# yeyupiaoling/PPASR

Hardware: AMD Instinct MI355X
Metric: audio-seconds/s (RTF^-1) Conformer-streaming fbank, batch32 per GPU, ctc_greedy (higher is better)
Workload: dtype f32; 1 GPU; configs[1]: Conformer streaming (configs/conformer.yml), fbank-80, 32 x 10 s utterances per GPU, V=4233, ctc_greedy, features resident in HBM -> token ids + scores on device; global_batch=32, frames=1000, decoder=ctc_greedy, parallelism=utterance-dp1, pipelined=False, gemm=f32

## Files before the change

### ppasr_amd/csrc/conformer_kernels.hip

```cpp
#include <cstdlib>

#include "conformer_kernels.h"
#include "launch.h"
#include "phases.h"
#include "h3.h"

#include <math.h>

namespace ppasr {
#ifdef PPASR_PHASE_TS
}
extern "C" __attribute__((visibility("default"))) int ppasr_debug_read_phase_ts(long long* out) {
  return (int)hipMemcpyFromSymbol(out, HIP_SYMBOL(ppasr::g_phase_ts), sizeof(long long) * 128);
}
extern "C" __attribute__((visibility("default"))) int ppasr_debug_read_wave_ts(long long* out) {
  return (int)hipMemcpyFromSymbol(out, HIP_SYMBOL(ppasr::g_wave_ts), sizeof(long long) * 512);
}
extern "C" __attribute__((visibility("default"))) int ppasr_debug_read_wg_ts(long long* out) {
  return (int)hipMemcpyFromSymbol(out, HIP_SYMBOL(ppasr::g_wg_ts), sizeof(long long) * 2 * 1024);
}
namespace ppasr {
#endif


// ... 26 lines not shown
  }
};
struct QkvStoreSide {
  const f32x16& acc;
  float* out;
  const f32x4 (&bias)[4];
  __device__ __forceinline__ void operator()(int g) const {
    if ((g & 7) == 4 && out) {
      const int q = g >> 3;
      *reinterpret_cast<f32x4*>(out + 8 * q) = f32x4{acc[4 * q] + bias[q][0], acc[4 * q + 1] + bias[q][1],
                                                     acc[4 * q + 2] + bias[q][2], acc[4 * q + 3] + bias[q][3]};
    }
  }
};

template <bool H3 = false>
__device__ __forceinline__ void ffn_qkv_body(float* bufX, float* bufA, float* bufH, float* __restrict__ x1,
                                             float* __restrict__ qkv, const LayerW& w, int r0, int valid, int n_chunks,
                                             BRing<1>& ring, VtOut vt = VtOut{}) {
  const int lane = lane_id(), wave = wave_id();
  rb_layernorm(bufX, bufA, kLda, kRows, w.ln_mac_g, w.ln_mac_b, 1e-5f);
  __syncthreads();
  PPASR_TS(8);
  f32x16 acc2[1][1];
  acc_zero(acc2);
  const f32x4* wq = w.wqkv + (size_t)wave * kTs256;
  if constexpr (H3) ffn_phase_h3(bufA, w.ffm_w1, w.ffm_b1, w.ffm_w2, n_chunks, wq, ring, acc2);
  else ffn_phase<true>(bufA, bufH, w.ffm_w1, w.ffm_b1, w.ffm_w2, n_chunks, wq, ring, acc2);
  PPASR_TS(9);
  residual_epilogue_t(bufX, acc2, w.ffm_b2, 0.5f);
  __syncthreads();
  PPASR_TS(10);
  rb_store_rows(x1 + (size_t)r0 * kD, bufX, kLda, kRows, valid);
  rb_layernorm(bufX, bufA, kLda, kRows, w.ln_mha_g, w.ln_mha_b, 1e-5f);
  __syncthreads();
  if constexpr (H3) h3_planes_from_tile(bufA, reinterpret_cast<_Float16*>(bufA));
  PPASR_TS(11);
  f32x16 tile[3][1][1]; bool qk_bad = false;
  const int cq = wave * 32 + 4 * (lane >> 5);
  float* qrow = (lane & 31) < valid ? qkv + (size_t)(r0 + (lane & 31)) * 768 + cq : nullptr;
  f32x4 qb[2][4], kp[4];
#pragma unroll
  for (int c = 0; c < 3; ++c)
#pragma unroll
    for (int q = 0; q < 4; ++q) (c < 2 ? qb[c][q] : kp[q]) = qkv_bias_quad<H3>(w.bqkv, vt, c, r0 + (lane & 31), cq + 8 * q);
#pragma unroll
  for (int c = 0; c < 3; ++c) {
    acc_zero(tile[c]);
    const f32x4* seg = w.wqkv + (size_t)(c * 8 + wave) * kTs256;
    const f32x4* nseg = c < 2 ? seg + 8 * kTs256 : nullptr;
    if constexpr (H3) {
      const _Float16* pa = reinterpret_cast<const _Float16*>(bufA);
      if (c < 2)
        rb_gemm_h3(pa, seg, nseg, ring, tile[c][0][0]);
      else
        rb_gemm_h3_rows<1, 16, QkStoreTailH3>(pa, kLdh, kPlaneH, seg, nseg, ring, tile[c],
                                              QkStoreTailH3{tile[0][0][0], tile[1][0][0], qrow, qb, vt.k_h3 != 0, qk_bad, cq});
    } else if (c == 0) {
      rb_gemm<1, 1, kG256, kPF, NoSide, true>(bufA, kLda, seg, 0, nseg, 0, ring, tile[c]);
    } else if (c == 1) {
      rb_gemm<1, 1, kG256, kPF, QkvStoreSide, true>(bufA, kLda, seg, 0, nseg, 0, ring, tile[c],
                                                    QkvStoreSide{tile[0][0][0], qrow, qb[0]});
    } else {
      rb_gemm<1, 1, kG256, kPF, QkvStoreSide, false>(bufA, kLda, seg, 0, nseg, 0, ring, tile[c],
                                                     QkvStoreSide{tile[1][0][0], qrow ? qrow + 256 : nullptr, qb[1]});
    }
    if (c == 0) qkv_kpos_add<H3>(qb[1], kp, vt);
    PPASR_TS(12 + c);
  }
  if constexpr (H3) h3_note(qk_bad);
  if (vt.vt) {
    const float bv = w.bqkv[2 * 256 + wave * 32 + (lane & 31)];
    float* dst = vt.vt + ((size_t)wave * (vt.stride >> 3) + (r0 >> 3)) * 256 + 4 * lane;
    if constexpr (H3) tile[2][0][0] *= kH3Inv;
#pragma unroll
    for (int i = 0; i < 4; ++i) {
      const f32x16& t = tile[2][0][0];
      *reinterpret_cast<f32x4*>(dst + i * 256) = f32x4{t[4 * i] + bv, t[4 * i + 1] + bv, t[4 * i + 2] + bv, t[4 * i + 3] + bv};
    }
  } else {
    const int col = 2 * 256 + wave * 32 + (lane & 31);
    const float bv = w.bqkv[col];
    if constexpr (H3) tile[2][0][0] *= kH3Inv;
#pragma unroll
    for (int r = 0; r < 16; ++r) {
      int row = acc_row(r, lane);
      if (row < valid) qkv[(size_t)(r0 + row) * 768 + col] = tile[2][0][0][r] + bv;
    }
  }
}

__global__ __launch_bounds__(kThreads) void k_ffn_qkv(const float* __restrict__ x_in, float* __restrict__ x1,
                                                      float* __restrict__ qkv, LayerW w, int M, int n_chunks, PadSkip ps,
                                                      VtOut vt) {
  extern __shared__ __attribute__((aligned(16))) float smem[];
  const int blk = pad_block_of(ps, kRows, M);
  if (blk < 0) return;
  float* bufX = smem;
  float* bufA = bufX + kRows * kLda;
  float* bufH = bufA + kRows * kLda;
  const int wave = wave_id();
  const int r0 = blk * kRows;
  const int valid = min(kRows, M - r0);
  BRing<1> ring;
  ring_prime(ring, w.ffm_w1 + (size_t)wave * kTs256, 0);
  rb_load_rows(bufX, kLda, x_in + (size_t)r0 * kD, kRows, valid);
  ffn_qkv_body(bufX, bufA, bufH, x1, qkv, w, r0, valid, n_chunks, ring, vt);
}
__global__ __launch_bounds__(256) void k_repack_h3(const float* __restrict__ src, _Float16* __restrict__ dst, int n_tiles, int G,
                                                   unsigned int* __restrict__ ovf) {
  const int KS = G >> 1;
  const long long t = (long long)blockIdx.x * 256 + threadIdx.x;
  if (t >= (long long)n_tiles * KS * 64) return;
  const int l = (int)(t & 63), ks = (int)((t >> 6) % KS), nt = (int)((t >> 6) / KS);
  const float* g = src + ((size_t)nt * G + 2 * ks + (l >> 5)) * 256;
  f16x8 hi, lo;
#pragma unroll
  for (int e = 0; e < 8; ++e) {
    const float v = g[((l & 31) + 32 * (e >> 2)) * 4 + (e & 3)] * kH3Sw;
    if (!(fabsf(v) <= kH3Max)) atomicAdd(ovf, 1u);
    hi[e] = (_Float16)v;
    lo[e] = (_Float16)(v - (float)hi[e]);
// ... 29 lines not shown
__global__ __launch_bounds__(kThreads) void k_ffn_qkv_h3(const float* __restrict__ x_in, float* __restrict__ x1,
                                                         float* __restrict__ qkv, LayerW w, int M, int n_chunks, PadSkip ps,
                                                         VtOut vt) {
  extern __shared__ __attribute__((aligned(16))) float smem[];
  const int blk = pad_block_of(ps, kRows, M);
  if (blk < 0) return;
  float* bufX = smem;
  float* bufA = bufX + kRows * kLda;
  float* bufH = bufA + kRows * kLda;
  const int wave = wave_id();
  const int r0 = blk * kRows;
  const int valid = min(kRows, M - r0);
  BRing<1> ring;
  ring_prime(ring, w.ffm_w1 + (size_t)wave * kTs256, 0);
  rb_load_rows(bufX, kLda, x_in + (size_t)r0 * kD, kRows, valid);
  ffn_qkv_body<true>(bufX, bufA, bufH, x1, qkv, w, r0, valid, n_chunks, ring, vt);
}
static void check_form(const char* stage, int rows, bool only32) {
  if (rows == 32 || ((rows == 16 || rows == kW16) && !only32)) return;
  fprintf(stderr, "ppasr_hip: %s refused: row-block form %d%s\n", stage, rows,
          only32 ? " with h3, g_hist, xhat_out, split_xhat or hm (8-wave 32-row form only)" : " (32, 16 or kW16)");
  abort();
}
constexpr size_t kLdsFfnQkv = 4 * kRows * kLda * sizeof(float);
void launch_ffn_qkv(const float* x_in, float* x1, float* qkv, const LayerW& w, int M, int n_chunks, hipStream_t st,
                    const PadSkip& ps, VtOut vt, bool h3, int rows) {
  check_form("launch_ffn_qkv", rows, h3);
  if (rows == 16) return LayerStagesT<16>::ffn_qkv(x_in, x1, qkv, w, M, n_chunks, st, ps, VtOut{});
  if (rows == kW16) return LayerStagesT<kW16>::ffn_qkv(x_in, x1, qkv, w, M, n_chunks, st, ps, vt);
  if (h3) {
    PPASR_LAUNCH(k_ffn_qkv_h3, dim3((M + kRows - 1) / kRows), dim3(kThreads), kLdsFfnQkv + kH3ExtraLds, st, x_in, x1, qkv, w,
                 M, n_chunks, ps, vt);
    return;
  }
  PPASR_LAUNCH(k_ffn_qkv, dim3((M + kRows - 1) / kRows), dim3(kThreads), kLdsFfnQkv, st, x_in, x1, qkv, w, M,
                     n_chunks, ps, vt);
}

void launch_attention(const AttnArgs& a, int B, int H, hipStream_t st) {
// ... 135 lines not shown
  if (split_xhat) {
    if (h3)
      PPASR_LAUNCH(k_pw1_glu_cols<true>, dim3(grid.x, 2), dim3(kThreads), kLdsPw1Cols + 512, st, xh, g, w, M, ps);
    else
      PPASR_LAUNCH(k_pw1_glu_cols<false>, dim3(grid.x, 2), dim3(kThreads), kLdsPw1Cols, st, xh, g, w, M, ps);
  }
}

constexpr int kPLd = 68;
constexpr int kPTile = 32 * kPLd;
constexpr int kFusedAttnFloats = kWaves * kPTile + kWaves * 64 + kRows * kLda;
static_assert(2 * kRows * kLda <= kWaves * kPTile + kWaves * 64, "bufX/bufA alias the attention scratch");
static_assert(kRows * kLda + 128 + 4 * kPTile <= kWaves * kPTile, "the d rows (fp16 x3: the Q'_v planes, 512 B longer) and the four merge tiles fit in front of Stat");
static_assert(kH3TileBytes <= kRows * kLda * 4 + 512, "fp16 x3: the Q'_u planes at bufC run 512 B past it (the launch asks for them)");
static_assert(kRows * kLda * 4 + kH3TileBytes <= kWaves * kPTile * 4, "fp16 x3: operand planes at bufA stay in front of Stat");
static_assert(kFusedAttnFloats * 4 <= 160 * 1024, "LDS budget");
template <bool H3>
__device__ __forceinline__ void attn_out_glu_body(const AttnArgs& a, int B, const float* __restrict__ x1, float* __restrict__ x2,
                                                  float* __restrict__ g, const LayerW& w) {
  extern __shared__ __attribute__((aligned(16))) float smem[];
  float* Ps = smem;
  float* Stat = Ps + kWaves * kPTile;
  float* bufC = Stat + kWaves * 64;
  float* bufX = smem;
  float* bufA = bufX + kRows * kLda;
  const int lane = lane_id(), wave = wave_id();
  const int h = wave >> 1, khalf = wave & 1;
  const int nq = (a.T1 + 31) / 32;
  const int slot = blockIdx.x >> 3;
  const int b = (slot / nq) * 8 + (blockIdx.x & 7);
  const int q0 = (slot % nq) * 32;
  if (b >= B) return;
  const int T = a.T1;
  const int valid = min(32, T - q0);
  const float* __restrict__ qb = a.q + (size_t)b * T * a.q_stride;
  const float* __restrict__ kbp = a.k + (size_t)b * a.T2 * a.k_stride;
  const float* __restrict__ vbp = a.v + (size_t)b * a.T2 * a.v_stride;
  const float* __restrict__ ptab = a.ptab + (size_t)a.pos0 * kD;
  const int pstride = a.pos_stride;
  const int64_t len_b = a.lens ? a.lens[b] : (int64_t)a.mask_mul * a.T2;
// ... 65 lines not shown
      if constexpr (H3) {
        f16x4 hi, lo;
        h3_split4((v + pu) * kH3Sa, hi, lo, bad);
        _Float16* pu_pl = reinterpret_cast<_Float16*>(bufC) + row * kLdh + 4 * lane;
        *reinterpret_cast<f16x4*>(pu_pl) = hi;
        *reinterpret_cast<f16x4*>(pu_pl + kPlaneH) = lo;
        h3_split4((v + pv) * kH3Sa, hi, lo, bad);
        _Float16* pv_pl = reinterpret_cast<_Float16*>(QV) + row * kLdh + 4 * lane;
        *reinterpret_cast<f16x4*>(pv_pl) = hi;
        *reinterpret_cast<f16x4*>(pv_pl + kPlaneH) = lo;
      } else {
        *reinterpret_cast<f32x4*>(bufC + row * kLda + 4 * lane) = v + pu;
      }
    }
    if constexpr (H3) h3_note(bad);
    __syncthreads();
  }
  const float* qfrag_u = bufC + l31 * kLda + h * 64 + 4 * hh;
  auto qfrag = [&](int gk) -> f32x4 { return *reinterpret_cast<const f32x4*>(qfrag_u + 8 * gk); };
  PPASR_TS(33);
  if (khalf * 128 < U) prime_k(khalf * 128);
  f32x16 acc_o[2];
#pragma unroll
  for (int t = 0; t < 2; ++t)
#pragma unroll
    for (int r = 0; r < 16; ++r) acc_o[t][r] = 0.f;
  float m_run = -INFINITY, l_run = 0.f;
  bool first = true;

  const int nkb = (U + 255) / 256;
  for (int kb = 0; kb < nkb; ++kb) {
// ... 189 lines not shown
    if constexpr (!H3) {
#pragma unroll
      for (int q = 0; q < 4; ++q) res[q] = *reinterpret_cast<const f32x4*>(x1 + grow + cq + 8 * q);
    }
    f32x16 acc[1][1];
    acc_zero(acc);
    if constexpr (H3) {
      h3_planes_from_tile(bufC, reinterpret_cast<_Float16*>(bufA));
      rb_gemm_h3(reinterpret_cast<const _Float16*>(bufA), seg_o, seg_val, ring, acc[0][0]);
      acc[0][0] *= kH3Inv;
    } else {
      rb_gemm<1, 1, kG256, kPF, NoSide, true>(bufC, kLda, seg_o, 0, seg_val, 0, ring, acc);
    }
#pragma unroll
    for (int q = 0; q < 4; ++q) {
      const f32x4 bo = *reinterpret_cast<const f32x4*>(w.bo + cq + 8 * q);
      f32x4 v;
#pragma unroll
      for (int e = 0; e < 4; ++e) v[e] = res[q][e] + (acc[0][0][4 * q + e] + bo[e]);
      if constexpr (H3) x2v[q] = v;
      else if (row_ok) *reinterpret_cast<f32x4*>(x2 + grow + cq + 8 * q) = v;
      if (!row_ok) v = f32x4{0.f, 0.f, 0.f, 0.f};
      *reinterpret_cast<f32x4*>(bufX + l31 * kLda + cq + 8 * q) = v;
    }
  }
  __syncthreads();
  PPASR_TS(37);
  struct PadHere {
    int64_t len_b;
    int q0, mul;
    __device__ __forceinline__ bool operator()(int row) const { return (int64_t)mul * (q0 + row) >= len_b; }
  };
  rb_layernorm<false>(bufX, bufA, kLda, kRows, w.ln_conv_g, w.ln_conv_b, 1e-5f,
                      PadHere{a.lens ? len_b : (int64_t)1 << 62, q0, a.mask_mul});
  __syncthreads();
  PPASR_TS(38);
  {
    f32x16 av[1][1], ag[1][1];
    acc_zero(av);
    acc_zero(ag);
    if constexpr (H3) {
      h3_planes_from_tile(bufA, reinterpret_cast<_Float16*>(bufA));
      rb_gemm_h3(reinterpret_cast<const _Float16*>(bufA), seg_val, seg_gate, ring, av[0][0]);
      rb_gemm_h3(reinterpret_cast<const _Float16*>(bufA), seg_gate, nullptr, ring, ag[0][0]);
      av[0][0] *= kH3Inv;
      ag[0][0] *= kH3Inv;
    } else {
      rb_gemm<1, 1, kG256, kPF, NoSide, true>(bufA, kLda, seg_val, 0, seg_gate, 0, ring, av);
      rb_gemm<1, 1, kG256, kPF, NoSide, true>(bufA, kLda, seg_gate, 0, nullptr, 0, ring, ag);
    }
#pragma unroll
    for (int q = 0; q < 4; ++q) {
      const f32x4 bval = *reinterpret_cast<const f32x4*>(w.pw1_b + cq + 8 * q);
      const f32x4 bgate = *reinterpret_cast<const f32x4*>(w.pw1_b + kD + cq + 8 * q);
      const f32x2 s0 = sigmoid2(f32x2{ag[0][0][4 * q] + bgate[0], ag[0][0][4 * q + 1] + bgate[1]});
      const f32x2 s1 = sigmoid2(f32x2{ag[0][0][4 * q + 2] + bgate[2], ag[0][0][4 * q + 3] + bgate[3]});
      const f32x4 o = {(av[0][0][4 * q] + bval[0]) * s0[0], (av[0][0][4 * q + 1] + bval[1]) * s0[1],
                       (av[0][0][4 * q + 2] + bval[2]) * s1[0], (av[0][0][4 * q + 3] + bval[3]) * s1[1]};
      if (row_ok) *reinterpret_cast<f32x4*>(g + grow + cq + 8 * q) = o;
    }
    if constexpr (H3) {
      if (row_ok) {
#pragma unroll
        for (int q = 0; q < 4; ++q) *reinterpret_cast<f32x4*>(x2 + grow + cq + 8 * q) = x2v[q];
      }
    }
  }
  PPASR_TS(39);
  PPASR_WG_TS(512 + 1);
}
__global__ __launch_bounds__(kThreads) void k_attn_out_glu(AttnArgs a, int B, const float* __restrict__ x1,
                                                           float* __restrict__ x2, float* __restrict__ g, LayerW w) {
  attn_out_glu_body<false>(a, B, x1, x2, g, w);
}
__global__ __launch_bounds__(kThreads) void k_attn_out_glu_h3(AttnArgs a, int B, const float* __restrict__ x1,
                                                              float* __restrict__ x2, float* __restrict__ g, LayerW w) {
  attn_out_glu_body<true>(a, B, x1, x2, g, w);
}
constexpr size_t kLdsAttnOutGlu = (size_t)kFusedAttnFloats * sizeof(float);
void launch_attn_out_glu(const AttnArgs& a, int B, const float* x1, float* x2, float* g, const LayerW& w, hipStream_t st, bool h3) {
  const int nq = (a.T1 + 31) / 32;
  if (h3)
    PPASR_LAUNCH(k_attn_out_glu_h3, dim3(nq * ((B + 7) / 8) * 8), dim3(kThreads), kLdsAttnOutGlu + 512, st, a, B, x1, x2, g, w);
  else
    PPASR_LAUNCH(k_attn_out_glu, dim3(nq * ((B + 7) / 8) * 8), dim3(kThreads), kLdsAttnOutGlu, st, a, B, x1, x2, g, w);
}

template <int KS, bool STREAM, bool NEXT, bool H3>
__device__ __forceinline__ void conv_ffn_body(const float* __restrict__ g, const float* __restrict__ g_hist,
                                              const float* __restrict__ x2, float* __restrict__ x_out, const LayerW& w,
                                              const int64_t* __restrict__ lens, int M, int Tp, int n_chunks, int mask_mul,
                                              const LayerW& wn, float* __restrict__ x1_next, float* __restrict__ qkv_next,
                                              int left_ctx, const PadSkip& ps, VtOut vt_next) {
  extern __shared__ __attribute__((aligned(16))) float smem[];
  const int blk = pad_block_of(ps, kRows, M);
  if (blk < 0) return;
  float* bufX = smem;
  float* bufA = bufX + kRows * kLda;
  float* bufH = bufA + kRows * kLda;
  const int lane = lane_id(), wave = wave_id();
  const int r0 = blk * kRows;
  const int valid = min(kRows, M - r0);
  const int col = wave * 32 + (lane & 31);
  BRing<1> ring;
  const f32x4* seg_pw2 = w.pw2 + (size_t)wave * kTs256;
  PPASR_TS(0);
  if (NEXT) PPASR_WG_TS(0);
  ring_prime(ring, seg_pw2, 0);
  const int pb0 = r0 / Tp, pt0 = r0 - pb0 * Tp, pnb = max(M / Tp, 1);
  int64_t plen0 = 0, plen1 = 0;
  if (lens && Tp >= kRows) {
    plen0 = lens[min(pb0, pnb - 1)];
    plen1 = lens[min(pb0 + 1, pnb - 1)];
  }
  if (!STREAM && KS <= 15 && Tp >= kRows / kWaves) {
    if constexpr (!STREAM && KS <= 15)
      dwconv_ln_phase<KS>(g, bufA, w.dw_w, w.dw_b, w.glu_pad, w.ln_cm_g, w.ln_cm_b, w.cm_eps, r0, M, Tp, left_ctx);
    PPASR_TS(1);
// ... 10 lines not shown
    const float* rp = x2 + (size_t)(r0 + min(l31, valid - 1)) * kD + cq;
#pragma unroll
    for (int q = 0; q < 4; ++q) res[q] = *reinterpret_cast<const f32x4*>(rp + 8 * q);
  }
  bool pad = false;
  if (lens) {
    if (Tp >= kRows) {
      const int tt = pt0 + l31;
      const bool over = tt >= Tp;
      const int64_t t = over ? tt - Tp : tt, len = over ? plen1 : plen0;
      pad = r0 + l31 < M && (int64_t)mask_mul * t >= len;
    } else {
      pad = is_pad(l31);
    }
  }
  __syncthreads();
  PPASR_TS(2);
  {
    f32x16 acc[1][1];
    acc_zero(acc);
    if constexpr (H3) {
      h3_planes_from_tile(bufA, reinterpret_cast<_Float16*>(bufA));
      rb_gemm_h3(reinterpret_cast<const _Float16*>(bufA), seg_pw2, w.ff_w1 + (size_t)wave * kTs256, ring, acc[0][0]);
      acc[0][0] *= kH3Inv;
    } else {
      rb_gemm<1, 1, kG256, kPF, NoSide, true>(bufA, kLda, seg_pw2, 0, w.ff_w1 + (size_t)wave * kTs256, 0, ring, acc);
    }
#pragma unroll
    for (int q = 0; q < 4; ++q) {
      const f32x4 bv = *reinterpret_cast<const f32x4*>(w.pw2_b + cq + 8 * q);
      f32x4 o;
#pragma unroll
      for (int e = 0; e < 4; ++e) o[e] = (l31 < valid) ? res[q][e] + (pad ? 0.f : acc[0][0][4 * q + e] + bv[e]) : 0.f;
      *reinterpret_cast<f32x4*>(bufX + l31 * kLda + cq + 8 * q) = o;
    }
  }
  __syncthreads();
  PPASR_TS(3);
  rb_layernorm(bufX, bufA, kLda, kRows, w.ln_ff_g, w.ln_ff_b, 1e-5f);
  __syncthreads();
  PPASR_TS(4);
  f32x16 acc2[1][1];
  acc_zero(acc2);
  if constexpr (H3)
    ffn_phase_h3(bufA, w.ff_w1, w.ff_b1, w.ff_w2, n_chunks, NEXT ? wn.ffm_w1 + (size_t)wave * kTs256 : nullptr, ring, acc2);
  else
    ffn_phase<true>(bufA, bufH, w.ff_w1, w.ff_b1, w.ff_w2, n_chunks, NEXT ? wn.ffm_w1 + (size_t)wave * kTs256 : nullptr,
                    ring, acc2);
  PPASR_TS(5);
  residual_epilogue_t(bufX, acc2, w.ff_b2, 0.5f);
  __syncthreads();
  PPASR_TS(6);
  rb_layernorm(bufX, bufX, kLda, kRows, w.ln_fin_g, w.ln_fin_b, 1e-5f);
  if (x_out) rb_store_rows(x_out + (size_t)r0 * kD, bufX, kLda, kRows, valid);
  PPASR_TS(7);
  if (NEXT) ffn_qkv_body<H3>(bufX, bufA, bufH, x1_next, qkv_next, wn, r0, valid, n_chunks, ring, vt_next);
  PPASR_TS(15);
  if (NEXT) PPASR_WG_TS(1);
}
template <int KS, bool STREAM, bool NEXT>
__global__ __launch_bounds__(kThreads) void k_conv_ffn(const float* __restrict__ g, const float* __restrict__ g_hist,
                                                       const float* __restrict__ x2, float* __restrict__ x_out, LayerW w,
                                                       const int64_t* __restrict__ lens, int M, int Tp, int n_chunks,
                                                       int mask_mul, LayerW wn, float* __restrict__ x1_next,
                                                       float* __restrict__ qkv_next, int left_ctx, PadSkip ps, VtOut vt_next) {
  conv_ffn_body<KS, STREAM, NEXT, false>(g, g_hist, x2, x_out, w, lens, M, Tp, n_chunks, mask_mul, wn, x1_next, qkv_next,
                                         left_ctx, ps, vt_next);
}
template <int KS, bool NEXT>
__global__ __launch_bounds__(kThreads) void k_conv_ffn_h3(const float* __restrict__ g, const float* __restrict__ x2,
                                                          float* __restrict__ x_out, LayerW w, const int64_t* __restrict__ lens,
                                                          int M, int Tp, int n_chunks, int mask_mul, LayerW wn,
                                                          float* __restrict__ x1_next, float* __restrict__ qkv_next,
                                                          int left_ctx, PadSkip ps, VtOut vt_next) {
  conv_ffn_body<KS, false, NEXT, true>(g, nullptr, x2, x_out, w, lens, M, Tp, n_chunks, mask_mul, wn, x1_next, qkv_next,
                                       left_ctx, ps, vt_next);
}
constexpr size_t kLdsConvFfn = 4 * kRows * kLda * sizeof(float);
void launch_conv_ffn(const float* g, const float* g_hist, const float* x2, float* x_out, const LayerW& w,
                     const int64_t* lens, int M, int Tp, int n_chunks, int ksize, int mask_mul, const LayerW* next,
                     float* x1_next, float* qkv_next, hipStream_t st, bool causal, const PadSkip& ps, VtOut vt_next, bool h3,
                     int rows) {
  check_form("launch_conv_ffn", rows, h3 || g_hist);
  if (rows == 16)
    return LayerStagesT<16>::conv_ffn(g, x2, x_out, w, lens, M, Tp, n_chunks, ksize, mask_mul, next, x1_next, qkv_next, st,
                                      causal, ps, VtOut{});
  if (rows == kW16)
    return LayerStagesT<kW16>::conv_ffn(g, x2, x_out, w, lens, M, Tp, n_chunks, ksize, mask_mul, next, x1_next, qkv_next, st,
                                        causal, ps, vt_next);
  dim3 grid((M + kRows - 1) / kRows);
  const int left_ctx = causal ? ksize - 1 : (ksize - 1) / 2;
  const LayerW& wn = next ? *next : w;
  if (h3) {
// ... 108 lines not shown
    residual_epilogue_t(bufX, acc2, w.ff_b2, 0.5f);
  } else {
    ffn_phase(bufA, bufH, w.ff_w1, w.ff_b1, w.ff_w2, n_chunks, nullptr, ring, acc2);
    residual_epilogue(bufX, acc2, w.ff_b2, 0.5f);
  }
  __syncthreads();
  rb_layernorm(bufX, bufX, kLda, kRows, w.ln_fin_g, w.ln_fin_b, 1e-5f);
  rb_store_rows(x_out + (size_t)r0 * kD, bufX, kLda, kRows, valid);
}
void launch_conv_ffn_stride(const float* g, const float* g_hist, const float* x2, float* x_out, const LayerW& w,
                            const int64_t* lens, int B, int Tp, int Ts, int n_chunks, int ksize, int mask_mul_out,
                            hipStream_t st, const PadSkip& ps, bool causal, bool h3, float* x3_out) {
  dim3 grid((B * Ts + kRows - 1) / kRows);
  (void)ksize;
  if (h3)
    PPASR_LAUNCH((k_conv_ffn_stride<15, true>), grid, dim3(kThreads), kLdsConvFfn + kH3ExtraLds, st, g, g_hist, x2, x_out, w, lens,
                 B, Tp, Ts, n_chunks, mask_mul_out, ps, causal ? 1 : 0, x3_out);
  else
    PPASR_LAUNCH((k_conv_ffn_stride<15, false>), grid, dim3(kThreads), kLdsConvFfn, st, g, g_hist, x2, x_out, w, lens, B, Tp, Ts,
                 n_chunks, mask_mul_out, ps, causal ? 1 : 0, x3_out);
}

hipError_t configure_kernels() {
  hipError_t e = configure_attention_kernels();
  if (e != hipSuccess) return e;
  e = configure_conformer_t_kernels();
  if (e != hipSuccess) return e;
  e = configure_front_fused_kernels();
  if (e != hipSuccess) return e;
  e = configure_front_kernels();
  if (e != hipSuccess) return e;
  e = configure_stream_kernels();
  if (e != hipSuccess) return e;
  e = configure_split_route_kernels();
// ... 12 lines not shown
  SET_LDS(k_out_glu<false>, kLdsOutGlu);
  SET_LDS(k_out_glu<true>, kLdsOutGlu + 512);
  SET_LDS(k_pw1_glu_cols<false>, kLdsPw1Cols);
  SET_LDS(k_pw1_glu_cols<true>, kLdsPw1Cols + 512);
  SET_LDS((k_conv_ffn<15, false, false>), kLdsConvFfn);
  SET_LDS((k_conv_ffn<31, false, false>), kLdsConvFfn);
  SET_LDS((k_conv_ffn<7, false, false>), kLdsConvFfn);
  SET_LDS((k_conv_ffn<15, false, true>), kLdsConvFfn);
  SET_LDS((k_conv_ffn<31, false, true>), kLdsConvFfn);
  SET_LDS((k_conv_ffn<7, false, true>), kLdsConvFfn);
  SET_LDS((k_conv_ffn<15, true, false>), kLdsConvFfn);
  SET_LDS((k_conv_ffn<31, true, false>), kLdsConvFfn);
  SET_LDS((k_conv_ffn<7, true, false>), kLdsConvFfn);
  SET_LDS(k_attn_out_glu, kLdsAttnOutGlu);
  SET_LDS(k_attn_out_glu_h3, kLdsAttnOutGlu + 512);
  SET_LDS((k_conv_ffn_stride<15, false>), kLdsConvFfn);
  SET_LDS((k_conv_ffn_stride<15, true>), kLdsConvFfn + kH3ExtraLds);
#undef SET_LDS
  return hipSuccess;
}

}
```

### ppasr_amd/csrc/phases.h

```cpp
#pragma once
#include "conformer_kernels.h"
#include "rowblock.h"

namespace ppasr {

struct SwishSide {
  const f32x16& acc;
  float* dst;
  const f32x4 (&bias)[4];
  mutable f32x2 lo;
  __device__ __forceinline__ void operator()(int g) const {
    const int q = g >> 3;
    if ((g & 7) == 0) lo = swish2(f32x2{acc[4 * q] + bias[q][0], acc[4 * q + 1] + bias[q][1]});
    if ((g & 7) == 4) {
      const f32x2 hi = swish2(f32x2{acc[4 * q + 2] + bias[q][2], acc[4 * q + 3] + bias[q][3]});
      *reinterpret_cast<f32x4*>(dst + 8 * q) = f32x4{lo[0], lo[1], hi[0], hi[1]};
    }
  }
};

template <bool T2 = false>
__device__ __forceinline__ void ffn_phase(const float* bufA, float* bufH, const f32x4* __restrict__ w1,
                                          const float* __restrict__ b1, const f32x4* __restrict__ w2, int n_chunks,
                                          const f32x4* __restrict__ after, BRing<1>& ring, f32x16 (&acc2)[1][1],
// ... 35 lines not shown
  }
}

__device__ __forceinline__ void residual_epilogue(float* bufX, const f32x16 (&acc)[1][1], const float* __restrict__ bias,
                                                  float scale) {
  const int lane = lane_id(), wave = wave_id();
  const int col = wave * 32 + (lane & 31);
  const float bv = bias[col];
#pragma unroll
  for (int r = 0; r < 16; ++r) {
    float* p = bufX + acc_row(r, lane) * kLda + col;
    *p = *p + scale * (acc[0][0][r] + bv);
  }
}

__device__ __forceinline__ void residual_epilogue_t(float* bufX, const f32x16 (&acc)[1][1], const float* __restrict__ bias,
                                                    float scale) {
  const int lane = lane_id(), wave = wave_id();
  const int cq = wave * 32 + 4 * (lane >> 5);
  float* row = bufX + (lane & 31) * kLda + cq;
#pragma unroll
  for (int q = 0; q < 4; ++q) {
    const f32x4 bv = *reinterpret_cast<const f32x4*>(bias + cq + 8 * q);
    f32x4 x = *reinterpret_cast<const f32x4*>(row + 8 * q);
#pragma unroll
    for (int e = 0; e < 4; ++e) x[e] = x[e] + scale * (acc[0][0][4 * q + e] + bv[e]);
    *reinterpret_cast<f32x4*>(row + 8 * q) = x;
  }
}

struct PadRows {
  const int64_t* lens;
  int r0, Tp, M;
  int mul = 4;
  __device__ __forceinline__ bool operator()(int row) const {
    if (!lens) return false;
    int m = r0 + row;
    if (m >= M) return false;
    int b = m / Tp, t = m - b * Tp;
    return mul * (int64_t)t >= lens[b];
  }
};
// ... 40 lines not shown
      acc += wj * xv;
    }
    *reinterpret_cast<f32x4*>(bufA + row * kLda + 4 * lane) = acc;
  }
}

template <int KS>
__device__ __forceinline__ void dwconv_ln_phase(const float* __restrict__ g, float* bufA, const float* __restrict__ dw_w,
                                                const float* __restrict__ dw_b, const float* __restrict__ glu_pad,
                                                const float* __restrict__ ln_g, const float* __restrict__ ln_b, float ln_eps, int r0,
                                                int M, int Tp, int left) {
  const int lane = lane_id(), wave = wave_id();
  constexpr int LO = KS - 1, RW = kRows / kWaves, NW = RW + LO;
  const bool causal = (left == LO);
  const int q0 = wave * RW;
  f32x4 x[NW];
#pragma unroll
  for (int q = 0; q < NW; ++q) {
    const int mq = r0 - left + q0 + q;
    const int mc = min(max(mq, 0), M - 1);
    const f32x4 v = *reinterpret_cast<const f32x4*>(g + (size_t)mc * kD + 4 * lane);
    x[q] = (mq >= 0 && mq < M) ? v : f32x4{0.f, 0.f, 0.f, 0.f};
  }
  f32x4 wt[KS];
#pragma unroll
  for (int j = 0; j < KS; ++j) wt[j] = *reinterpret_cast<const f32x4*>(dw_w + j * kD + 4 * lane);
  f32x4 gp = *reinterpret_cast<const f32x4*>(glu_pad + 4 * lane);
  if (!causal) gp = f32x4{0.f, 0.f, 0.f, 0.f};
  const f32x4 bias = *reinterpret_cast<const f32x4*>(dw_b + 4 * lane);
  const int m0 = r0 + q0;
  const int tq0 = m0 - (m0 / Tp) * Tp;
  const int npass = (tq0 + RW - 1 < Tp) ? 1 : 2;
  f32x4 out[RW];
#pragma unroll 1
  for (int p = 0; p < npass; ++p) {
    const int tqp = tq0 - p * Tp;
    f32x4 acc[RW];
#pragma unroll
    for (int i = 0; i < RW; ++i) acc[i] = bias;
#pragma unroll
    for (int q = 0; q < NW; ++q) {
      const int tt = tqp - left + q;
      const f32x4 xq = (tt >= 0 && tt < Tp) ? x[q] : gp;
#pragma unroll
      for (int i = 0; i < RW; ++i) {
        const int j = q - i;
        if (j >= 0 && j < KS) acc[i] += wt[j] * xq;
      }
    }
#pragma unroll
    for (int i = 0; i < RW; ++i)
      if (npass == 1 || (tqp + i >= 0 && tqp + i < Tp)) out[i] = acc[i];
  }
  const f32x4 gam = *reinterpret_cast<const f32x4*>(ln_g + 4 * lane);
  const f32x4 bet = *reinterpret_cast<const f32x4*>(ln_b + 4 * lane);
  ln_rows_inreg<true, RW>(out, gam, bet, ln_eps);
#pragma unroll
  for (int i = 0; i < RW; ++i) *reinterpret_cast<f32x4*>(bufA + (q0 + i) * kLda + 4 * lane) = out[i];
}

template <bool H3>
__device__ __forceinline__ f32x4 qkv_bias_quad(const float* __restrict__ bqkv, const VtOut& vt, int c, int m, int col) {
  if (c < 2) return *reinterpret_cast<const f32x4*>(bqkv + c * 256 + col);
  if constexpr (!H3) {
    if (vt.kpos) return *reinterpret_cast<const f32x4*>(vt.kpos + (size_t)(m - m / vt.Ti * vt.Ti) * vt.kpos_stride + col);
  }
  return f32x4{0.f, 0.f, 0.f, 0.f};
}
template <bool H3>
__device__ __forceinline__ void qkv_kpos_add(f32x4 (&bk)[4], const f32x4 (&kp)[4], const VtOut& vt) {
// ... 34 lines not shown
```

### ppasr_amd/csrc/rowblock.h

```cpp
#pragma once
#include <hip/hip_runtime.h>
#include <stdint.h>

typedef float f32x16 __attribute__((ext_vector_type(16)));
typedef float f32x4 __attribute__((ext_vector_type(4)));
typedef float f32x2 __attribute__((ext_vector_type(2)));

__device__ __forceinline__ float max3f(float a, float b, float c) {
  float d;
  asm volatile("v_max3_f32 %0, %1, %2, %3" : "=v"(d) : "v"(a), "v"(b), "v"(c));
  return d;
}

namespace ppasr {

constexpr int kD = 256;
constexpr int kLda = kD + 4;
constexpr int kRows = 32;
constexpr int kWaves = 8;
constexpr int kThreads = 64 * kWaves;
constexpr int kW16 = 1032;
constexpr int form_rows(int form) { return form == kW16 ? 32 : form; }
constexpr int kG256 = kD / 8;
constexpr int kTs256 = kG256 * 64;
// ... 200 lines not shown
    x[i] = x[i] - mean[i];
    var[i] = wave_sum(x[i][0] * x[i][0] + x[i][1] * x[i][1] + x[i][2] * x[i][2] + x[i][3] * x[i][3]) * (1.0f / kD);
  }
#pragma unroll
  for (int i = 0; i < RN; ++i) {
    const float rstd = 1.0f / sqrtf(var[i] + eps);
    x[i] = x[i] * rstd * g + b;
    if (SWISH) {
#pragma unroll
      for (int e = 0; e < 4; ++e) x[i][e] = swishf(x[i][e]);
    }
  }
}

template <bool SWISH = false, typename ZeroRow = NoZero>
__device__ __forceinline__ void rb_layernorm(const float* src, float* dst, int lda, int nrows,
                                             const float* __restrict__ gamma, const float* __restrict__ beta,
                                             float eps, ZeroRow zero_row = ZeroRow()) {
  const int lane = lane_id();
  const f32x4 g = *reinterpret_cast<const f32x4*>(gamma + 4 * lane);
  const f32x4 b = *reinterpret_cast<const f32x4*>(beta + 4 * lane);
  constexpr int RN = kRows / kWaves;
  if (nrows == kRows) {
    f32x4 x[RN];
#pragma unroll
    for (int i = 0; i < RN; ++i) x[i] = *reinterpret_cast<const f32x4*>(src + (wave_id() + i * kWaves) * lda + 4 * lane);
    ln_rows_inreg<SWISH, RN>(x, g, b, eps);
#pragma unroll
    for (int i = 0; i < RN; ++i) {
      const int row = wave_id() + i * kWaves;
      if (zero_row(row)) x[i] = f32x4{0.f, 0.f, 0.f, 0.f};
      *reinterpret_cast<f32x4*>(dst + row * lda + 4 * lane) = x[i];
    }
    return;
  }
  for (int row = wave_id(); row < nrows; row += kWaves) {
    f32x4 x[1];
    x[0] = *reinterpret_cast<const f32x4*>(src + row * lda + 4 * lane);
    ln_rows_inreg<SWISH, 1>(x, g, b, eps);
    if (zero_row(row)) x[0] = f32x4{0.f, 0.f, 0.f, 0.f};
    *reinterpret_cast<f32x4*>(dst + row * lda + 4 * lane) = x[0];
  }
}

__device__ __forceinline__ void rb_load_rows(float* dst, int lda, const float* __restrict__ src, int nrows, int valid) {
  const int lane = lane_id();
  for (int row = wave_id(); row < nrows; row += kWaves) {
    f32x4 v = {0.f, 0.f, 0.f, 0.f};
    if (row < valid) v = *reinterpret_cast<const f32x4*>(src + (size_t)row * kD + 4 * lane);
    *reinterpret_cast<f32x4*>(dst + row * lda + 4 * lane) = v;
  }
}

__device__ __forceinline__ void rb_store_rows(float* __restrict__ dst, const float* src, int lda, int nrows, int valid) {
  const int lane = lane_id();
  for (int row = wave_id(); row < nrows && row < valid; row += kWaves)
    *reinterpret_cast<f32x4*>(dst + (size_t)row * kD + 4 * lane) =
        *reinterpret_cast<const f32x4*>(src + row * lda + 4 * lane);
// ... 4 lines not shown
```

Measured before the change: 58390 audio-s/s.

## Stage per-layer bias and LayerNorm vectors into LDS early in fused kernels

Adds a small LDS region per fused layer kernel. Each wave issues global loads for the bias and LayerNorm gamma/beta vectors at kernel start, or during an earlier phase, and commits them to LDS at an existing barrier, so later epilogues read from LDS instead of issuing dependent global loads on the critical path. In the conv depthwise path the weight and LN-parameter loads are hoisted ahead of the input loads, with a scheduling barrier and the masking moved after the loads. The cost is extra LDS per block, which may reduce occupancy, plus more live registers holding the staged vectors.

```diff
diff --git a/ppasr_amd/csrc/conformer_kernels.hip b/ppasr_amd/csrc/conformer_kernels.hip
--- a/ppasr_amd/csrc/conformer_kernels.hip
+++ b/ppasr_amd/csrc/conformer_kernels.hip
@@ -64,12 +64,12 @@
   }
 };
 
-template <bool H3 = false>
+template <bool H3, bool STAGE>
 __device__ __forceinline__ void ffn_qkv_body(float* bufX, float* bufA, float* bufH, float* __restrict__ x1,
                                              float* __restrict__ qkv, const LayerW& w, int r0, int valid, int n_chunks,
-                                             BRing<1>& ring, VtOut vt = VtOut{}) {
+                                             BRing<1>& ring, VtOut vt, float* vec) {
   const int lane = lane_id(), wave = wave_id();
-  rb_layernorm(bufX, bufA, kLda, kRows, w.ln_mac_g, w.ln_mac_b, 1e-5f);
+  s1_first_layernorm<STAGE>(bufX, bufA, w, vec);
   __syncthreads();
   PPASR_TS(8);
   f32x16 acc2[1][1];
@@ -78,11 +78,11 @@
   if constexpr (H3) ffn_phase_h3(bufA, w.ffm_w1, w.ffm_b1, w.ffm_w2, n_chunks, wq, ring, acc2);
   else ffn_phase<true>(bufA, bufH, w.ffm_w1, w.ffm_b1, w.ffm_w2, n_chunks, wq, ring, acc2);
   PPASR_TS(9);
-  residual_epilogue_t(bufX, acc2, w.ffm_b2, 0.5f);
+  residual_epilogue_tv(bufX, acc2, vec + kVFfmB2 * kD, 0.5f);
   __syncthreads();
   PPASR_TS(10);
   rb_store_rows(x1 + (size_t)r0 * kD, bufX, kLda, kRows, valid);
-  rb_layernorm(bufX, bufA, kLda, kRows, w.ln_mha_g, w.ln_mha_b, 1e-5f);
+  rb_layernorm_v(bufX, bufA, vec + kVLnMhaG * kD, 1e-5f);
   __syncthreads();
   if constexpr (H3) h3_planes_from_tile(bufA, reinterpret_cast<_Float16*>(bufA));
   PPASR_TS(11);
@@ -93,7 +93,7 @@
 #pragma unroll
   for (int c = 0; c < 3; ++c)
 #pragma unroll
-    for (int q = 0; q < 4; ++q) (c < 2 ? qb[c][q] : kp[q]) = qkv_bias_quad<H3>(w.bqkv, vt, c, r0 + (lane & 31), cq + 8 * q);
+    for (int q = 0; q < 4; ++q) (c < 2 ? qb[c][q] : kp[q]) = qkv_bias_quad<H3>(vec + kVBq * kD, vt, c, r0 + (lane & 31), cq + 8 * q);
 #pragma unroll
   for (int c = 0; c < 3; ++c) {
     acc_zero(tile[c]);
@@ -120,7 +120,7 @@
   }
   if constexpr (H3) h3_note(qk_bad);
   if (vt.vt) {
-    const float bv = w.bqkv[2 * 256 + wave * 32 + (lane & 31)];
+    const float bv = vec[kVBv * kD + wave * 32 + (lane & 31)];
     float* dst = vt.vt + ((size_t)wave * (vt.stride >> 3) + (r0 >> 3)) * 256 + 4 * lane;
     if constexpr (H3) tile[2][0][0] *= kH3Inv;
 #pragma unroll
@@ -130,7 +130,7 @@
     }
   } else {
     const int col = 2 * 256 + wave * 32 + (lane & 31);
-    const float bv = w.bqkv[col];
+    const float bv = vec[kVBv * kD + wave * 32 + (lane & 31)];
     if constexpr (H3) tile[2][0][0] *= kH3Inv;
 #pragma unroll
     for (int r = 0; r < 16; ++r) {
@@ -155,7 +155,7 @@
   BRing<1> ring;
   ring_prime(ring, w.ffm_w1 + (size_t)wave * kTs256, 0);
   rb_load_rows(bufX, kLda, x_in + (size_t)r0 * kD, kRows, valid);
-  ffn_qkv_body(bufX, bufA, bufH, x1, qkv, w, r0, valid, n_chunks, ring, vt);
+  ffn_qkv_body<false, true>(bufX, bufA, bufH, x1, qkv, w, r0, valid, n_chunks, ring, vt, layer_vec(smem, 0));
 }
 __global__ __launch_bounds__(256) void k_repack_h3(const float* __restrict__ src, _Float16* __restrict__ dst, int n_tiles, int G,
                                                    unsigned int* __restrict__ ovf) {
@@ -215,7 +215,7 @@
   BRing<1> ring;
   ring_prime(ring, w.ffm_w1 + (size_t)wave * kTs256, 0);
   rb_load_rows(bufX, kLda, x_in + (size_t)r0 * kD, kRows, valid);
-  ffn_qkv_body<true>(bufX, bufA, bufH, x1, qkv, w, r0, valid, n_chunks, ring, vt);
+  ffn_qkv_body<true, true>(bufX, bufA, bufH, x1, qkv, w, r0, valid, n_chunks, ring, vt, layer_vec(smem, kH3ExtraLds));
 }
 static void check_form(const char* stage, int rows, bool only32) {
   if (rows == 32 || ((rows == 16 || rows == kW16) && !only32)) return;
@@ -223,7 +223,7 @@
           only32 ? " with h3, g_hist, xhat_out, split_xhat or hm (8-wave 32-row form only)" : " (32, 16 or kW16)");
   abort();
 }
-constexpr size_t kLdsFfnQkv = 4 * kRows * kLda * sizeof(float);
+constexpr size_t kLdsFfnQkv = kLdsLayerTiles + kVecS1 * kD * sizeof(float);
 void launch_ffn_qkv(const float* x_in, float* x1, float* qkv, const LayerW& w, int M, int n_chunks, hipStream_t st,
                     const PadSkip& ps, VtOut vt, bool h3, int rows) {
   check_form("launch_ffn_qkv", rows, h3);
@@ -389,7 +389,7 @@
 static_assert(kRows * kLda + 128 + 4 * kPTile <= kWaves * kPTile, "the d rows (fp16 x3: the Q'_v planes, 512 B longer) and the four merge tiles fit in front of Stat");
 static_assert(kH3TileBytes <= kRows * kLda * 4 + 512, "fp16 x3: the Q'_u planes at bufC run 512 B past it (the launch asks for them)");
 static_assert(kRows * kLda * 4 + kH3TileBytes <= kWaves * kPTile * 4, "fp16 x3: operand planes at bufA stay in front of Stat");
-static_assert(kFusedAttnFloats * 4 <= 160 * 1024, "LDS budget");
+static_assert((kFusedAttnFloats + kVecAttn * kD) * 4 + 512 <= 160 * 1024, "LDS budget (with the staged rows of the tail)");
 template <bool H3>
 __device__ __forceinline__ void attn_out_glu_body(const AttnArgs& a, int B, const float* __restrict__ x1, float* __restrict__ x2,
                                                   float* __restrict__ g, const LayerW& w) {
@@ -397,8 +397,8 @@
   float* Ps = smem;
   float* Stat = Ps + kWaves * kPTile;
   float* bufC = Stat + kWaves * 64;
-  float* bufX = smem;
-  float* bufA = bufX + kRows * kLda;
+  float *bufX = smem, *bufA = bufX + kRows * kLda;
+  AttnTailVecs tv(smem + kFusedAttnFloats + (H3 ? 128 : 0), w);
   const int lane = lane_id(), wave = wave_id();
   const int h = wave >> 1, khalf = wave & 1;
   const int nq = (a.T1 + 31) / 32;
@@ -494,7 +494,7 @@
       }
     }
     if constexpr (H3) h3_note(bad);
-    __syncthreads();
+    tv.commit_and_barrier();
   }
   const float* qfrag_u = bufC + l31 * kLda + h * 64 + 4 * hh;
   auto qfrag = [&](int gk) -> f32x4 { return *reinterpret_cast<const f32x4*>(qfrag_u + 8 * gk); };
@@ -714,7 +714,7 @@
     }
 #pragma unroll
     for (int q = 0; q < 4; ++q) {
-      const f32x4 bo = *reinterpret_cast<const f32x4*>(w.bo + cq + 8 * q);
+      const f32x4 bo = vec_quad(tv.vec + kVBo * kD, cq + 8 * q);
       f32x4 v;
 #pragma unroll
       for (int e = 0; e < 4; ++e) v[e] = res[q][e] + (acc[0][0][4 * q + e] + bo[e]);
@@ -731,8 +731,8 @@
     int q0, mul;
     __device__ __forceinline__ bool operator()(int row) const { return (int64_t)mul * (q0 + row) >= len_b; }
   };
-  rb_layernorm<false>(bufX, bufA, kLda, kRows, w.ln_conv_g, w.ln_conv_b, 1e-5f,
-                      PadHere{a.lens ? len_b : (int64_t)1 << 62, q0, a.mask_mul});
+  rb_layernorm_v<false>(bufX, bufA, tv.vec + kVLnConvG * kD, 1e-5f,
+                        PadHere{a.lens ? len_b : (int64_t)1 << 62, q0, a.mask_mul});
   __syncthreads();
   PPASR_TS(38);
   {
@@ -751,8 +751,8 @@
     }
 #pragma unroll
     for (int q = 0; q < 4; ++q) {
-      const f32x4 bval = *reinterpret_cast<const f32x4*>(w.pw1_b + cq + 8 * q);
-      const f32x4 bgate = *reinterpret_cast<const f32x4*>(w.pw1_b + kD + cq + 8 * q);
+      const f32x4 bval = vec_quad(tv.vec + kVPw1BVal * kD, cq + 8 * q);
+      const f32x4 bgate = vec_quad(tv.vec + kVPw1BGate * kD, cq + 8 * q);
       const f32x2 s0 = sigmoid2(f32x2{ag[0][0][4 * q] + bgate[0], ag[0][0][4 * q + 1] + bgate[1]});
       const f32x2 s1 = sigmoid2(f32x2{ag[0][0][4 * q + 2] + bgate[2], ag[0][0][4 * q + 3] + bgate[3]});
       const f32x4 o = {(av[0][0][4 * q] + bval[0]) * s0[0], (av[0][0][4 * q + 1] + bval[1]) * s0[1],
@@ -777,7 +777,7 @@
                                                               float* __restrict__ x2, float* __restrict__ g, LayerW w) {
   attn_out_glu_body<true>(a, B, x1, x2, g, w);
 }
-constexpr size_t kLdsAttnOutGlu = (size_t)kFusedAttnFloats * sizeof(float);
+constexpr size_t kLdsAttnOutGlu = (size_t)(kFusedAttnFloats + kVecAttn * kD) * sizeof(float);
 void launch_attn_out_glu(const AttnArgs& a, int B, const float* x1, float* x2, float* g, const LayerW& w, hipStream_t st, bool h3) {
   const int nq = (a.T1 + 31) / 32;
   if (h3)
@@ -801,7 +801,7 @@
   const int lane = lane_id(), wave = wave_id();
   const int r0 = blk * kRows;
   const int valid = min(kRows, M - r0);
-  const int col = wave * 32 + (lane & 31);
+  ConvFfnVecs<NEXT> sv(layer_vec(smem, H3 ? kH3ExtraLds : 0), w, wn);
   BRing<1> ring;
   const f32x4* seg_pw2 = w.pw2 + (size_t)wave * kTs256;
   PPASR_TS(0);
@@ -842,7 +842,7 @@
       pad = is_pad(l31);
     }
   }
-  __syncthreads();
+  sv.commit_and_barrier();
   PPASR_TS(2);
   {
     f32x16 acc[1][1];
@@ -856,7 +856,7 @@
     }
 #pragma unroll
     for (int q = 0; q < 4; ++q) {
-      const f32x4 bv = *reinterpret_cast<const f32x4*>(w.pw2_b + cq + 8 * q);
+      const f32x4 bv = vec_quad(sv.vec + kVPw2B * kD, cq + 8 * q);
       f32x4 o;
 #pragma unroll
       for (int e = 0; e < 4; ++e) o[e] = (l31 < valid) ? res[q][e] + (pad ? 0.f : acc[0][0][4 * q + e] + bv[e]) : 0.f;
@@ -865,7 +865,7 @@
   }
   __syncthreads();
   PPASR_TS(3);
-  rb_layernorm(bufX, bufA, kLda, kRows, w.ln_ff_g, w.ln_ff_b, 1e-5f);
+  rb_layernorm_v(bufX, bufA, sv.vec + kVLnFfG * kD, 1e-5f);
   __syncthreads();
   PPASR_TS(4);
   f32x16 acc2[1][1];
@@ -876,13 +876,13 @@
     ffn_phase<true>(bufA, bufH, w.ff_w1, w.ff_b1, w.ff_w2, n_chunks, NEXT ? wn.ffm_w1 + (size_t)wave * kTs256 : nullptr,
                     ring, acc2);
   PPASR_TS(5);
-  residual_epilogue_t(bufX, acc2, w.ff_b2, 0.5f);
+  residual_epilogue_tv(bufX, acc2, sv.vec + kVFfB2 * kD, 0.5f);
   __syncthreads();
   PPASR_TS(6);
-  rb_layernorm(bufX, bufX, kLda, kRows, w.ln_fin_g, w.ln_fin_b, 1e-5f);
+  rb_layernorm_v(bufX, bufX, sv.vec + kVLnFinG * kD, 1e-5f);
   if (x_out) rb_store_rows(x_out + (size_t)r0 * kD, bufX, kLda, kRows, valid);
   PPASR_TS(7);
-  if (NEXT) ffn_qkv_body<H3>(bufX, bufA, bufH, x1_next, qkv_next, wn, r0, valid, n_chunks, ring, vt_next);
+  if (NEXT) ffn_qkv_body<H3, false>(bufX, bufA, bufH, x1_next, qkv_next, wn, r0, valid, n_chunks, ring, vt_next, sv.vec);
   PPASR_TS(15);
   if (NEXT) PPASR_WG_TS(1);
 }
@@ -904,7 +904,7 @@
   conv_ffn_body<KS, false, NEXT, true>(g, nullptr, x2, x_out, w, lens, M, Tp, n_chunks, mask_mul, wn, x1_next, qkv_next,
                                        left_ctx, ps, vt_next);
 }
-constexpr size_t kLdsConvFfn = 4 * kRows * kLda * sizeof(float);
+constexpr size_t kLdsConvFfn = kLdsLayerTiles + kVecConvFfn * kD * sizeof(float);
 void launch_conv_ffn(const float* g, const float* g_hist, const float* x2, float* x_out, const LayerW& w,
                      const int64_t* lens, int M, int Tp, int n_chunks, int ksize, int mask_mul, const LayerW* next,
                      float* x1_next, float* qkv_next, hipStream_t st, bool causal, const PadSkip& ps, VtOut vt_next, bool h3,
@@ -1043,10 +1043,10 @@
   dim3 grid((B * Ts + kRows - 1) / kRows);
   (void)ksize;
   if (h3)
-    PPASR_LAUNCH((k_conv_ffn_stride<15, true>), grid, dim3(kThreads), kLdsConvFfn + kH3ExtraLds, st, g, g_hist, x2, x_out, w, lens,
+    PPASR_LAUNCH((k_conv_ffn_stride<15, true>), grid, dim3(kThreads), kLdsLayerTiles + kH3ExtraLds, st, g, g_hist, x2, x_out, w, lens,
                  B, Tp, Ts, n_chunks, mask_mul_out, ps, causal ? 1 : 0, x3_out);
   else
-    PPASR_LAUNCH((k_conv_ffn_stride<15, false>), grid, dim3(kThreads), kLdsConvFfn, st, g, g_hist, x2, x_out, w, lens, B, Tp, Ts,
+    PPASR_LAUNCH((k_conv_ffn_stride<15, false>), grid, dim3(kThreads), kLdsLayerTiles, st, g, g_hist, x2, x_out, w, lens, B, Tp, Ts,
                  n_chunks, mask_mul_out, ps, causal ? 1 : 0, x3_out);
 }
 
@@ -1089,8 +1089,8 @@
   SET_LDS((k_conv_ffn<7, true, false>), kLdsConvFfn);
   SET_LDS(k_attn_out_glu, kLdsAttnOutGlu);
   SET_LDS(k_attn_out_glu_h3, kLdsAttnOutGlu + 512);
-  SET_LDS((k_conv_ffn_stride<15, false>), kLdsConvFfn);
-  SET_LDS((k_conv_ffn_stride<15, true>), kLdsConvFfn + kH3ExtraLds);
+  SET_LDS((k_conv_ffn_stride<15, false>), kLdsLayerTiles);
+  SET_LDS((k_conv_ffn_stride<15, true>), kLdsLayerTiles + kH3ExtraLds);
 #undef SET_LDS
   return hipSuccess;
 }
diff --git a/ppasr_amd/csrc/phases.h b/ppasr_amd/csrc/phases.h
--- a/ppasr_amd/csrc/phases.h
+++ b/ppasr_amd/csrc/phases.h
@@ -73,18 +73,86 @@
   }
 }
 
+__device__ __forceinline__ void residual_epilogue_tq(float* bufX, const f32x16 (&acc)[1][1], const f32x4 (&bv)[4], float scale) {
+  const int lane = lane_id(), wave = wave_id();
+  const int cq = wave * 32 + 4 * (lane >> 5);
+  float* row = bufX + (lane & 31) * kLda + cq;
+#pragma unroll
+  for (int q = 0; q < 4; ++q) {
+    f32x4 x = *reinterpret_cast<const f32x4*>(row + 8 * q);
+#pragma unroll
+    for (int e = 0; e < 4; ++e) x[e] = x[e] + scale * (acc[0][0][4 * q + e] + bv[q][e]);
+    *reinterpret_cast<f32x4*>(row + 8 * q) = x;
+  }
+}
 __device__ __forceinline__ void residual_epilogue_t(float* bufX, const f32x16 (&acc)[1][1], const float* __restrict__ bias,
                                                     float scale) {
-  const int lane = lane_id(), wave = wave_id();
-  const int cq = wave * 32 + 4 * (lane >> 5);
-  float* row = bufX + (lane & 31) * kLda + cq;
-#pragma unroll
-  for (int q = 0; q < 4; ++q) {
-    const f32x4 bv = *reinterpret_cast<const f32x4*>(bias + cq + 8 * q);
-    f32x4 x = *reinterpret_cast<const f32x4*>(row + 8 * q);
-#pragma unroll
-    for (int e = 0; e < 4; ++e) x[e] = x[e] + scale * (acc[0][0][4 * q + e] + bv[e]);
-    *reinterpret_cast<f32x4*>(row + 8 * q) = x;
+  const int cq = wave_id() * 32 + 4 * (lane_id() >> 5);
+  f32x4 bv[4];
+#pragma unroll
+  for (int q = 0; q < 4; ++q) bv[q] = *reinterpret_cast<const f32x4*>(bias + cq + 8 * q);
+  residual_epilogue_tq(bufX, acc, bv, scale);
+}
+
+enum VecRow {
+  kVLnMacG, kVLnMacB, kVFfmB2, kVLnMhaG, kVLnMhaB, kVBq, kVBk, kVBv, kVecS1,
+  kVPw2B = kVecS1, kVLnFfG, kVLnFfB, kVFfB2, kVLnFinG, kVLnFinB, kVecConvFfn
+};
+enum AttnVecRow { kVBo, kVLnConvG, kVLnConvB, kVPw1BVal, kVPw1BGate, kVecAttn };
+constexpr int kLayerTileFloats = 4 * kRows * kLda;
+constexpr size_t kLdsLayerTiles = kLayerTileFloats * sizeof(float);
+static_assert((kLayerTileFloats + kVecConvFfn * kD) * sizeof(float) + 2048 <= 160 * 1024, "LDS budget (fp16 x3 adds 1 536 B)");
+__device__ __forceinline__ float* layer_vec(float* smem, int extra_bytes) {
+  return smem + kLayerTileFloats + extra_bytes / (int)sizeof(float);
+}
+template <bool SWISH = false, typename ZeroRow = NoZero>
+__device__ __forceinline__ void rb_layernorm_v(const float* src, float* dst, const float* g_row, float eps,
+                                               ZeroRow zero_row = ZeroRow()) {
+  const int lane = lane_id();
+  rb_layernorm_gb<SWISH, ZeroRow>(src, dst, kLda, kRows, vec_quad(g_row, 4 * lane), vec_quad(g_row + kD, 4 * lane), eps, zero_row);
+}
+__device__ __forceinline__ void residual_epilogue_tv(float* bufX, const f32x16 (&acc)[1][1], const float* bias_row, float scale) {
+  f32x4 bv[4];
+  vec_quads(bv, bias_row, wave_id() * 32 + 4 * (lane_id() >> 5));
+  residual_epilogue_tq(bufX, acc, bv, scale);
+}
+template <bool NEXT>
+struct ConvFfnVecs {
+  static constexpr int V0 = NEXT ? 0 : kVecS1, NV = kVecConvFfn - V0;
+  float* vec;
+  VecStage<NV> stage;
+  __device__ __forceinline__ ConvFfnVecs(float* vec_, const LayerW& w, const LayerW& wn) : vec(vec_) {
+    if constexpr (NEXT)
+      vec_stage_request(stage, wn.ln_mac_g, wn.ln_mac_b, wn.ffm_b2, wn.ln_mha_g, wn.ln_mha_b, wn.bqkv, wn.bqkv + 256,
+                        wn.bqkv + 512, w.pw2_b, w.ln_ff_g, w.ln_ff_b, w.ff_b2, w.ln_fin_g, w.ln_fin_b);
+    else
+      vec_stage_request(stage, w.pw2_b, w.ln_ff_g, w.ln_ff_b, w.ff_b2, w.ln_fin_g, w.ln_fin_b);
+  }
+  __device__ __forceinline__ void commit_and_barrier() {
+    vec_stage_commit(vec + V0 * kD, stage);
+    __syncthreads();
+  }
+};
+struct AttnTailVecs {
+  float* vec;
+  VecStage<kVecAttn> stage;
+  __device__ __forceinline__ AttnTailVecs(float* vec_, const LayerW& w) : vec(vec_) {
+    vec_stage_request(stage, w.bo, w.ln_conv_g, w.ln_conv_b, w.pw1_b, w.pw1_b + kD);
+  }
+  __device__ __forceinline__ void commit_and_barrier() {
+    vec_stage_commit(vec, stage);
+    __syncthreads();
+  }
+};
+template <bool STAGE>
+__device__ __forceinline__ void s1_first_layernorm(const float* bufX, float* bufA, const LayerW& w, float* vec) {
+  if constexpr (STAGE) {
+    VecStage<kVecS1 - kVFfmB2> stage;
+    vec_stage_request(stage, w.ffm_b2, w.ln_mha_g, w.ln_mha_b, w.bqkv, w.bqkv + 256, w.bqkv + 512);
+    rb_layernorm(bufX, bufA, kLda, kRows, w.ln_mac_g, w.ln_mac_b, 1e-5f);
+    vec_stage_commit(vec + kVFfmB2 * kD, stage);
+  } else {
+    rb_layernorm_v(bufX, bufA, vec + kVLnMacG * kD, 1e-5f);
   }
 }
 
@@ -155,20 +223,27 @@
   constexpr int LO = KS - 1, RW = kRows / kWaves, NW = RW + LO;
   const bool causal = (left == LO);
   const int q0 = wave * RW;
+  f32x4 wt[KS];
+#pragma unroll
+  for (int j = 0; j < KS; ++j) wt[j] = *reinterpret_cast<const f32x4*>(dw_w + j * kD + 4 * lane);
+  f32x4 gp = *reinterpret_cast<const f32x4*>(glu_pad + 4 * lane);
+  const f32x4 bias = *reinterpret_cast<const f32x4*>(dw_b + 4 * lane);
+  const f32x4 gam = *reinterpret_cast<const f32x4*>(ln_g + 4 * lane);
+  const f32x4 bet = *reinterpret_cast<const f32x4*>(ln_b + 4 * lane);
   f32x4 x[NW];
 #pragma unroll
   for (int q = 0; q < NW; ++q) {
     const int mq = r0 - left + q0 + q;
     const int mc = min(max(mq, 0), M - 1);
-    const f32x4 v = *reinterpret_cast<const f32x4*>(g + (size_t)mc * kD + 4 * lane);
-    x[q] = (mq >= 0 && mq < M) ? v : f32x4{0.f, 0.f, 0.f, 0.f};
-  }
-  f32x4 wt[KS];
-#pragma unroll
-  for (int j = 0; j < KS; ++j) wt[j] = *reinterpret_cast<const f32x4*>(dw_w + j * kD + 4 * lane);
-  f32x4 gp = *reinterpret_cast<const f32x4*>(glu_pad + 4 * lane);
+    x[q] = *reinterpret_cast<const f32x4*>(g + (size_t)mc * kD + 4 * lane);
+  }
+  __builtin_amdgcn_sched_barrier(0);
   if (!causal) gp = f32x4{0.f, 0.f, 0.f, 0.f};
-  const f32x4 bias = *reinterpret_cast<const f32x4*>(dw_b + 4 * lane);
+#pragma unroll
+  for (int q = 0; q < NW; ++q) {
+    const int mq = r0 - left + q0 + q;
+    if (!(mq >= 0 && mq < M)) x[q] = f32x4{0.f, 0.f, 0.f, 0.f};
+  }
   const int m0 = r0 + q0;
   const int tq0 = m0 - (m0 / Tp) * Tp;
   const int npass = (tq0 + RW - 1 < Tp) ? 1 : 2;
@@ -193,8 +268,6 @@
     for (int i = 0; i < RW; ++i)
       if (npass == 1 || (tqp + i >= 0 && tqp + i < Tp)) out[i] = acc[i];
   }
-  const f32x4 gam = *reinterpret_cast<const f32x4*>(ln_g + 4 * lane);
-  const f32x4 bet = *reinterpret_cast<const f32x4*>(ln_b + 4 * lane);
   ln_rows_inreg<true, RW>(out, gam, bet, ln_eps);
 #pragma unroll
   for (int i = 0; i < RW; ++i) *reinterpret_cast<f32x4*>(bufA + (q0 + i) * kLda + 4 * lane) = out[i];
diff --git a/ppasr_amd/csrc/rowblock.h b/ppasr_amd/csrc/rowblock.h
--- a/ppasr_amd/csrc/rowblock.h
+++ b/ppasr_amd/csrc/rowblock.h
@@ -238,12 +238,9 @@
 }
 
 template <bool SWISH = false, typename ZeroRow = NoZero>
-__device__ __forceinline__ void rb_layernorm(const float* src, float* dst, int lda, int nrows,
-                                             const float* __restrict__ gamma, const float* __restrict__ beta,
-                                             float eps, ZeroRow zero_row = ZeroRow()) {
-  const int lane = lane_id();
-  const f32x4 g = *reinterpret_cast<const f32x4*>(gamma + 4 * lane);
-  const f32x4 b = *reinterpret_cast<const f32x4*>(beta + 4 * lane);
+__device__ __forceinline__ void rb_layernorm_gb(const float* src, float* dst, int lda, int nrows, const f32x4 g, const f32x4 b,
+                                                float eps, ZeroRow zero_row = ZeroRow()) {
+  const int lane = lane_id();
   constexpr int RN = kRows / kWaves;
   if (nrows == kRows) {
     f32x4 x[RN];
@@ -266,6 +263,48 @@
     *reinterpret_cast<f32x4*>(dst + row * lda + 4 * lane) = x[0];
   }
 }
+template <bool SWISH = false, typename ZeroRow = NoZero>
+__device__ __forceinline__ void rb_layernorm(const float* src, float* dst, int lda, int nrows,
+                                             const float* __restrict__ gamma, const float* __restrict__ beta,
+                                             float eps, ZeroRow zero_row = ZeroRow()) {
+  const int lane = lane_id();
+  const f32x4 g = *reinterpret_cast<const f32x4*>(gamma + 4 * lane);
+  const f32x4 b = *reinterpret_cast<const f32x4*>(beta + 4 * lane);
+  rb_layernorm_gb<SWISH, ZeroRow>(src, dst, lda, nrows, g, b, eps, zero_row);
+}
+
+template <int N>
+struct VecStage {
+  f32x4 v[(N + kWaves - 1) / kWaves];
+};
+__device__ __forceinline__ const float* vec_pick(int, const float* p0) { return p0; }
+template <typename... P>
+__device__ __forceinline__ const float* vec_pick(int r, const float* p0, P... rest) {
+  const float* q = vec_pick(r - 1, rest...);
+  return r == 0 ? p0 : q;
+}
+template <typename... P>
+__device__ __forceinline__ void vec_stage_request(VecStage<(int)sizeof...(P)>& s, P... rows) {
+  constexpr int N = (int)sizeof...(P);
+  const int lane = lane_id(), wave = wave_id();
+#pragma unroll
+  for (int i = 0; i * kWaves < N; ++i) {
+    const float* p = vec_pick(min(i * kWaves + wave, N - 1), rows...);
+    s.v[i] = *reinterpret_cast<const f32x4*>(p + 4 * lane);
+  }
+}
+template <int N>
+__device__ __forceinline__ void vec_stage_commit(float* vec, const VecStage<N>& s) {
+  const int lane = lane_id(), wave = wave_id();
+#pragma unroll
+  for (int i = 0; i * kWaves < N; ++i)
+    if (i * kWaves + wave < N) *reinterpret_cast<f32x4*>(vec + (i * kWaves + wave) * kD + 4 * lane) = s.v[i];
+}
+__device__ __forceinline__ f32x4 vec_quad(const float* row, int col) { return *reinterpret_cast<const f32x4*>(row + col); }
+__device__ __forceinline__ void vec_quads(f32x4 (&b)[4], const float* row, int cq) {
+#pragma unroll
+  for (int q = 0; q < 4; ++q) b[q] = vec_quad(row, cq + 8 * q);
+}
 
 __device__ __forceinline__ void rb_load_rows(float* dst, int lda, const float* __restrict__ src, int nrows, int valid) {
   const int lane = lane_id();
```

Result: no change. 58590 audio-s/s, median of 6 (+0.3%).
